# jaymarichua/Applestar

Hardware: AMD Instinct MI355X
Metric: learner samples/sec (AlphaStar policy) (higher is better)
Workload: dtype fp32

## Files before the change

applestar_amd/csrc/bindings.cpp:

```cpp
#include <cstring>
#include <cstdlib>
#include <map>
#include <string>
#include <torch/extension.h>
#include <c10/hip/HIPStream.h>
#include <c10/hip/HIPGuard.h>

#include "kernels.h"

namespace {

hipStream_t stream() { return c10::hip::getCurrentHIPStream().stream(); }

int dt(const at::Tensor& t) {
  if (t.scalar_type() == at::kFloat) return as::DT_F32;
  if (t.scalar_type() == at::kBFloat16) return as::DT_BF16;
  TORCH_CHECK(false, "applestar_amd: unsupported dtype ", t.scalar_type());
}

void check_cuda(const at::Tensor& t, const char* name) {
  TORCH_CHECK(t.is_cuda(), "applestar_amd: ", name, " must be a GPU tensor");
  TORCH_CHECK(t.is_contiguous(), "applestar_amd: ", name, " must be contiguous");
}

// ... 1634 lines not shown
  TORCH_CHECK(dy.dim() == 2, "wgrad: dy [R, N]");
  TORCH_CHECK(dy.is_contiguous() && x.is_contiguous(), "wgrad: dy and x must be contiguous");
  const int64_t R = dy.size(0), N = dy.size(1);
  int64_t K, H = 1, W = 1;
  if (cin > 0) {
    TORCH_CHECK(x.dim() == 4 && x.size(3) == cin && x.size(0) * x.size(1) * x.size(2) == R, "wgrad: x NHWC");
    H = x.size(1);
    W = x.size(2);
    K = 9 * cin;
    TORCH_CHECK(cin % 8 == 0, "wgrad: Cin % 8");
  } else {
    TORCH_CHECK(x.dim() == 2 && x.size(0) == R, "wgrad: x [R, K]");
    K = x.size(1);
  }
  TORCH_CHECK(N % 8 == 0 && K % 8 == 0, "wgrad: N and K must be multiples of 8");
  TORCH_CHECK(R * N * 2 < 0x7ffffff0LL && x.numel() * 2 < 0x7ffffff0LL, "wgrad: tensor too large");
  c10::hip::HIPGuard g(dy.device().index());
  const int S = R > 0 ? as::wgrad_splits(R, static_cast<int>(N), static_cast<int>(K)) : 1;
  auto opts = dy.options().dtype(at::kFloat);
  if (R == 0) {
    auto zo = bf16_out ? dy.options() : opts;
    return {at::zeros({N, K}, zo), want_bias ? at::zeros({N}, zo) : at::Tensor()};
  }
  const int64_t NK = N * K, stride = NK + (want_bias ? N : 0);
  if (bf16_out && S == 1) {
    auto flat = at::empty({stride}, dy.options());
    as::wgrad(dy.data_ptr(), x.data_ptr(), reinterpret_cast<float*>(flat.data_ptr()),
              want_bias ? reinterpret_cast<float*>(static_cast<at::BFloat16*>(flat.data_ptr()) + NK) : nullptr, 0, R,
              static_cast<int>(N), static_cast<int>(K), static_cast<int>(H), static_cast<int>(W), static_cast<int>(cin),
              1, stream(), true);
    return {flat.narrow(0, 0, NK).view({N, K}), want_bias ? flat.narrow(0, NK, N) : at::Tensor()};
  }
  auto part = at::empty({S, stride}, opts);
  static const bool nan_fill = [] {
    const char* e = std::getenv("APPLESTAR_WGRAD_NANFILL");
    return e != nullptr && e[0] == '1';
  }();
  if (nan_fill) part.fill_(std::numeric_limits<float>::quiet_NaN());
  as::wgrad(dy.data_ptr(), x.data_ptr(), part.data_ptr<float>(), want_bias ? part.data_ptr<float>() + NK : nullptr,
            stride, R, static_cast<int>(N), static_cast<int>(K), static_cast<int>(H), static_cast<int>(W),
            static_cast<int>(cin), S, stream());
  at::Tensor flat;
  if (bf16_out && S <= 1024) {
    flat = at::empty({stride}, dy.options());
    as::column_reduce_bf16(part.data_ptr<float>(), flat.data_ptr(), S, static_cast<int>(stride), stream());
  } else if (S == 1) {
    flat = part.view({stride});
  } else {
    flat = at::empty({stride}, opts);
    as::column_reduce(part.data_ptr<float>(), flat.data_ptr<float>(), S, static_cast<int>(stride), stream());
  }
  if (bf16_out && flat.scalar_type() != at::kBFloat16) flat = flat.to(at::kBFloat16);
  return {flat.narrow(0, 0, NK).view({N, K}), want_bias ? flat.narrow(0, NK, N) : at::Tensor()};
}

namespace {
int idx_code(const at::Tensor& t) {
  if (t.scalar_type() == at::kShort) return 0;
  if (t.scalar_type() == at::kInt) return 1;
  TORCH_CHECK(t.scalar_type() == at::kLong, "bo_encoder: index dtype int16 / int32 / int64");
  return 2;
}

as::BoWeights bo_weights(const std::vector<at::Tensor>& p, int* wdt) {
  TORCH_CHECK(p.size() == 2 + 12 * as::kBoLayers, "bo_encoder: 38 parameter tensors");
  const auto lin_t = p[0].scalar_type();
  TORCH_CHECK(lin_t == at::kFloat || lin_t == at::kBFloat16, "bo_encoder: linear dtype");
  auto lin = [&](const at::Tensor& t, int64_t numel) {
    TORCH_CHECK(t.is_cuda() && t.is_contiguous() && t.scalar_type() == lin_t && t.numel() == numel,
                "bo_encoder: linear parameter (dtype / shape / contiguity)");
    return static_cast<const void*>(t.data_ptr());
  };
  auto ln = [&](const at::Tensor& t) {
    TORCH_CHECK(t.is_cuda() && t.is_contiguous() && t.scalar_type() == at::kFloat && t.numel() == 64,
                "bo_encoder: LayerNorm parameter fp32 [64]");
    return t.data_ptr<float>();
  };
  as::BoWeights w;
  w.w0 = lin(p[0], 64 * 214);
  w.b0 = lin(p[1], 64);
  for (int l = 0; l < as::kBoLayers; ++l) {
    const int o = 2 + 12 * l;
    w.ln1w[l] = ln(p[o]);
    w.ln1b[l] = ln(p[o + 1]);
    w.wqkv[l] = lin(p[o + 2], 48 * 64);
    w.bqkv[l] = lin(p[o + 3], 48);
    w.wp[l] = lin(p[o + 4], 64 * 16);
    w.bp[l] = lin(p[o + 5], 64);
    w.ln2w[l] = ln(p[o + 6]);
    w.ln2b[l] = ln(p[o + 7]);
    w.w1[l] = lin(p[o + 8], 128 * 64);
    w.b1[l] = lin(p[o + 9], 128);
    w.w2[l] = lin(p[o + 10], 64 * 128);
    w.b2[l] = lin(p[o + 11], 64);
  }
  *wdt = lin_t == at::kBFloat16 ? as::DT_BF16 : as::DT_F32;
  return w;
}
}

std::vector<at::Tensor> bo_encoder_fwd(const at::Tensor& bo, const at::Tensor& loc, const std::vector<at::Tensor>& params,
                                       bool save) {
  check_cuda(bo, "bo");
  check_cuda(loc, "loc");
  TORCH_CHECK(bo.dim() == 2 && bo.size(1) == as::kBoTokens && bo.is_contiguous() && loc.sizes() == bo.sizes() &&
                  loc.is_contiguous() && loc.scalar_type() == bo.scalar_type(),
// ... 966 lines not shown
  m.def("varlen_attn_fwd_f32", &varlen_attn_fwd_f32);
  m.def("conv3x3_f32_epi2", &conv3x3_f32_epi2);
  m.def("conv3x3_f32_epi2_supported", &conv3x3_f32_epi2_supported);
  m.def("conv3x3_f32", &conv3x3_f32);
  m.def("fused_clip_adam", &fused_clip_adam);
  m.def("head_sample", &head_sample);
  m.def("target_unit_sample", &target_unit_sample);
  m.def("fused_adam_chunk", &as::fused_adam_chunk);
  m.def("wgrad_f32", &wgrad_f32, py::arg("dy"), py::arg("x"), py::arg("cin"), py::arg("want_bias"),
        py::arg("out") = py::none());
  m.def("gemm_f32", &gemm_f32);
  m.def("gemm_bf16_small", &gemm_bf16_small);
  m.def("gemm_bf16", &gemm_bf16);
  m.def("small_gemm", &small_gemm);
  m.def("small_wgrad", &small_wgrad);
  m.def("small_gemm_splitk", &small_gemm_splitk);
  m.def("f32_mfma_mode", &as::f32_mfma_mode);
  m.def("set_f32_pipe_variant", &as::set_f32_pipe_variant);
  m.def("set_f32_conv_variant", &as::set_f32_conv_variant);
  m.def("set_f32_mfma_mode", &as::set_f32_mfma_mode);
  m.def("conv3x3_f32_supported", &as::conv3x3_f32_supported);
  m.def("varlen_attn_bwd_f32", &varlen_attn_bwd_f32);
  m.def("attn_f32_variant", [](int64_t v) { return static_cast<int64_t>(as::attn_f32_variant(static_cast<int>(v))); });
  m.def("su_sample", &su_sample);
  m.def("segment_copy", &segment_copy);
  m.def("conv_wt", &conv_wt);
  m.def("upconv1_fwd", &upconv1_fwd);
  m.def("upconv1_bwd", &upconv1_bwd, py::arg("x_nhwc"), py::arg("w"), py::arg("dy"), py::arg("relu_mask") = false);
  m.def("maxpool2_fwd", &maxpool2_fwd);
  m.def("maxpool2_bwd", &maxpool2_bwd, py::arg("dy"), py::arg("pos"), py::arg("H"), py::arg("W"),
        py::arg("mask") = py::none());
  m.def("maxpool2_bwd_relu", &maxpool2_bwd_relu);
  m.def("spatial_embed_pool_fwd", &spatial_embed_pool_fwd, py::arg("planes"), py::arg("effects"), py::arg("w_dense"),
        py::arg("bias"), py::arg("rows"), py::arg("ex"), py::arg("ey"), py::arg("entity_num"),
        py::arg("ordered") = false);
  m.def("spatial_pool_supported", [](int64_t h, int64_t w) { return as::spatial_pool_supported(static_cast<int>(h), static_cast<int>(w)); });
  m.def("segment_sum", &segment_sum);
  m.def("spatial_dense_wgrad_pooled", &spatial_dense_wgrad_pooled);
  m.def("spatial_gather_rows_pooled", &spatial_gather_rows_pooled);
  m.def("entity_mean_pool", &entity_mean_pool);
  m.def("table_grad", &table_grad, py::arg("src"), py::arg("idx"), py::arg("V"), py::arg("ordered") = false);
  m.def("gather_steps_fwd", &gather_steps_fwd);
  m.def("gather_steps_bwd", &gather_steps_bwd);
  m.def("scatter_conn_fwd", &scatter_conn_fwd);
  m.def("scatter_conn_bwd", &scatter_conn_bwd);
  m.def("conv3x3_fwd", &conv3x3_fwd);
  m.def("wgrad", &wgrad, py::arg("dy"), py::arg("x"), py::arg("cin"), py::arg("want_bias"),
        py::arg("bf16_out") = false);
  m.def("pointwise_conv", &pointwise_conv);
  m.def("pointwise_supported", [](int64_t ci, int64_t co) { return as::pointwise_supported(static_cast<int>(ci), static_cast<int>(co)); });
  m.def("lstm_split_error", &lstm_split_error);
  m.def("lstm_split_flag", &lstm_split_flag);
  m.def("multi_copy", &multi_copy);
  m.def("ln_affine_grads", &ln_affine_grads);
  m.def("multi_strided_copy", &multi_strided_copy);
  m.def("multi_accumulate", &multi_accumulate);
  m.def("multi_strided_accumulate", &multi_strided_accumulate);
  m.def("loc_in_fwd", &loc_in_fwd);
  m.def("vsp_fwd", &vsp_fwd);
  m.def("rl_loss", &rl_loss, py::arg("alp"), py::arg("blp"), py::arg("hm"), py::arg("ent"), py::arg("kl"), py::arg("v"),
        py::arg("r"), py::arg("wm"), py::arg("atflag"), py::arg("sc"), py::arg("upgo_f"), py::arg("only_value"),
        py::arg("ordered") = false, py::arg("sk") = py::none(), py::arg("dflag") = py::none());
  m.def("sl_ce_fwd", &sl_ce_fwd, py::arg("logits"), py::arg("labels"), py::arg("eps"), py::arg("row_on") = py::none(),
        py::arg("su_len") = py::none(), py::arg("su_on") = py::none(), py::arg("S") = 1, py::arg("su_mask") = false);
  m.def("sl_ce_bwd", &sl_ce_bwd, py::arg("logits"), py::arg("labels"), py::arg("eps"), py::arg("row_on"),
        py::arg("su_len"), py::arg("su_on"), py::arg("S"), py::arg("su_mask"), py::arg("stats"), py::arg("grad"));
  m.def("sl_loss_tail", &sl_loss_tail, py::arg("losses"), py::arg("argmaxes"), py::arg("labels"), py::arg("masks"),
        py::arg("su_loss"), py::arg("su_labels"), py::arg("su_len"), py::arg("su_on"), py::arg("preds"),
        py::arg("ent_num"), py::arg("w"), py::arg("cr_scale"), py::arg("n"));
  m.def("sl_ce_su_max_c", []() { return as::sl_ce_su_max_c(); });
  m.def("gate_chain", &gate_chain);
  m.def("gate_chain_f32", &gate_chain_f32);
  m.def("vsp_pool_fwd", &vsp_pool_fwd);
  m.def("vsp_pool_bwd", &vsp_pool_bwd);
  m.def("vsp_in_channels", []() { return as::vsp_in_channels(); });
  m.def("vsp_out_channels", []() { return as::vsp_out_channels(); });
  m.def("vsp_bwd", &vsp_bwd);
  m.def("loc_in_supported", [](int64_t c, int64_t p) { return as::loc_in_supported(static_cast<int>(c), static_cast<int>(p)); });
  m.def("loc_in_bwd", &loc_in_bwd);
  m.def("head_stats_fwd", &head_stats_fwd, py::arg("logits"), py::arg("teacher"), py::arg("action"),
        py::arg("successive") = py::none());
  m.def("resmlp_fwd", &resmlp_fwd);
  m.def("resmlp_bwd", &resmlp_bwd);
  m.def("bo_encoder_fwd", &bo_encoder_fwd);
  m.def("bo_encoder_bwd", &bo_encoder_bwd, py::arg("bo"), py::arg("loc"), py::arg("params"), py::arg("save"),
        py::arg("dmean"), py::arg("ordered") = false);
  m.def("head_stats_bwd", &head_stats_bwd, py::arg("logits"), py::arg("teacher"), py::arg("action"), py::arg("stats"),
        py::arg("grad"), py::arg("successive") = py::none());
  m.def("act_grad_nhwc", &act_grad_nhwc);
  m.def("conv3x3_supported", [](int64_t cin, int64_t cout) { return as::conv3x3_supported(static_cast<int>(cin), static_cast<int>(cout)); });
}
```

applestar_amd/csrc/kernels.h:

```cpp
#pragma once
#include <hip/hip_runtime.h>
#include <stdint.h>

namespace as {

enum DType : int { DT_F32 = 0, DT_BF16 = 1 };
enum SrcType : int { SRC_U8 = 0, SRC_I8 = 1, SRC_I16 = 2, SRC_I32 = 3, SRC_I64 = 4, SRC_F16 = 5, SRC_F32 = 6 };
enum FieldKind : int { FIELD_ONE_HOT = 0, FIELD_BINARY = 1, FIELD_SCALAR = 2 };

constexpr int kMaxFields = 40;
struct EntityFields {
  const void* ptr[kMaxFields];
  int dtype[kMaxFields];
  int kind[kMaxFields];
  int offset[kMaxFields];
  int width[kMaxFields];
  int n;
};

void layer_norm_fwd(const void* x, int x_dt, const void* res, int res_dt, const float* w, const float* b,
                    void* y, int y_dt, float* xsum, float* mean, float* rstd, long rows, int cols, float eps,
                    int act, hipStream_t s);
void layer_norm_bwd(const void* dy, int dy_dt, const void* xin, int xin_dt, const void* y, int y_dt,
                    const float* w, const float* mean, const float* rstd, void* dx, int dx_dt,
                    float* dw_part, float* db_part, long rows, int cols, int act, int nblk, hipStream_t s,
                    const float* msrc = nullptr, float* dxm = nullptr);
void column_reduce(float* part, float* out, int nrows, int cols, hipStream_t s);
void entity_pack(const void* num, bool num64, int B, int N, long total, bool* valid, int64_t* flat, int64_t* seg,
                 int* cu, hipStream_t s);
void embed_relu_fwd(const void* table, int dt, const void* idx, int idt, void* out, long U, int V, int D,
                    hipStream_t s);
void embed_relu_bwd(const void* dout, const void* out, int dt, const void* idx, int idt, float* dtab, long U, int V,
                    int D, bool direct, hipStream_t s);
void column_reduce_bf16(const float* part, void* out, int nrows, int cols, hipStream_t s);
int layer_norm_bwd_blocks(long rows);

void reverse_scan(const float* a, const float* b, const float* init, float* y, int K, int T, int B,
                  hipStream_t s);

void gated_residual_fwd(const void* y, const void* g, const float* sp, const void* x, const void* post, void* out,
                        int dt, long n, hipStream_t s);
int vsp_in_channels();
int vsp_out_channels();
void vsp_fwd(const void* sc, const void* own, const void* enemy, const float* w, const float* b, void* out, long P,
             hipStream_t s, int dt = DT_BF16);
int vsp_bwd_blocks(long P);
void vsp_pool_fwd(const void* sc, const void* own, const void* enemy, const float* w, const float* b, void* pooled,
                  uint8_t* pos, int B, int H, int W, hipStream_t s, int dt = DT_BF16);
void vsp_pool_bwd(const void* dpooled, const uint8_t* pos, const void* pooled, const void* sc, const void* own,
                  const void* enemy, const float* w, void* dsc, float* part, int B, int H, int W, int nblk,
                  hipStream_t s, int dt = DT_BF16);
void vsp_bwd(const void* dout, const void* out, const void* sc, const void* own, const void* enemy, const float* w,
             void* dsc, float* part, long P, int nblk, hipStream_t s, int dt = DT_BF16);
bool loc_in_supported(int C, int P);
void loc_in_fwd(const void* y0, const void* p, const float* wp, void* out, long npix, int HW, hipStream_t s);
int loc_in_bwd_blocks(long npix);
void loc_in_bwd(const void* dy, const void* y, const void* p, const float* wp, void* dym, void* dp, float* part,
                long npix, int HW, int nblk, hipStream_t s);
void gated_residual_bwd(const void* dout, const void* y, const void* g, const float* sp, const void* out,
                        const void* xin, int dt, void* dy, void* dg, void* dx, float* dsp_part, long n, int nblk,
                        hipStream_t s);
int elementwise_blocks(long n);

bool lnlstm_supported(int H);
struct LstmSplit {
  unsigned long long* slab;
  int* err;
};
void lnlstm_fwd(const float* xp, const float* h0, const float* c0, const void* wT, int w_dt, const float* lnh_w,
                const float* lnh_b, const float* lnc_w, const float* lnc_b, int T, int B, int H, float eps, float* out,
                float* c_all, float* xhat_h, float* rstd_h, float* gates, float* xhat_c, float* rstd_c, float* hT,
                float* cT, hipStream_t s, const LstmSplit* split = nullptr, unsigned short* out_bf16 = nullptr);
void lnlstm_bwd(const float* dout, const float* dhT, const float* dcT, const float* gates, const float* c_all,
                const float* xhat_c, const float* rstd_c, const float* xhat_h, const float* rstd_h, const void* w,
                int w_dt, const float* lnh_w, const float* lnc_w, int T, int B, int H, float* dgates, float* dhg,
                float* dc_ln, float* dh0, float* dc0, hipStream_t s, const LstmSplit* split = nullptr);

void entity_embed_fwd(const EntityFields& f, const int64_t* index, const void* wT, int w_dt, const float* bias,
                      void* out, int out_dt, long T, hipStream_t s);
int entity_wgrad_chunks(long T);
void entity_embed_wgrad(const EntityFields& f, const int64_t* index, const void* dout, const void* out, int dt,
                        float* part, long T, int K_in, int nchunk, hipStream_t s);
void entity_onehot(const EntityFields& f, const int64_t* index, void* X, int x_dt, long T, int K_in, hipStream_t s);

struct SpatialPlanes {
  const uint8_t* height;
  const uint8_t* plane[6];
// ... 88 lines not shown
bool conv3x3_f32_supported(int Cin, int Cout);
void conv3x3_f32_fwd(const float* x, const float* w, const float* bias, const float* res, float* out, int B, int H,
                     int W, int Cin, int Cout, int act, hipStream_t s);
bool conv3x3_f32_epi2_supported(int Cin, int Cout);
void conv3x3_f32_fwd_epi2(const float* x, const float* w, const float* res, const float* res2, long res2_rows,
                          const float* mask, float* out, int B, int H, int W, int Cin, int Cout, hipStream_t s);
int wgrad_f32_splits(long R, int N, int K);
void set_f32_pipe_variant(int v);
int f32_conv_variant();
void set_f32_conv_variant(int v);
int f32_mfma_mode();
void set_f32_mfma_mode(int mode);
void small_nt(const void* a, const void* b, const float* bias, const void* res, const void* amask, int mask_mode,
              void* out, long M, int N, int K, int act, bool bf16, hipStream_t s);
int small_nt_splits(long M, int N, int K);
void small_nt_splitk(const void* a, const void* b, const float* bias, float* part, int S, void* out, long M, int N,
                     int K, int act, bool bf16, hipStream_t s);
void small_tn(const void* dy, const void* x, const void* ymask, int mask_mode, void* dw, void* db, long R, int N,
              int K, bool bf16_in, bool bf16_out, hipStream_t s);
void gemm_bf16_small(const void* a, const void* b, const float* bias, const void* res, void* out, long M, int N, int K,
                     int act, hipStream_t s);
bool gemm_f32_is_small(long M, int N);
void gemm_bf16(const void* a, const void* b, const float* bias, const void* res, void* out, long M, int N, int K,
               int act, hipStream_t s);
void gemm_f32(const float* a, const float* b, const float* bias, const float* res, float* out, long M, int N, int K,
              int act, hipStream_t s);
void wgrad_f32(const float* dy, const float* x, float* dw_part, float* db_part, long part_stride, long R, int N, int K,
               int H, int W, int Cin, int S, hipStream_t st);
int conv_wgrad_halo_f32_mode();
void set_conv_wgrad_halo_f32_mode(int mode);
bool conv_wgrad_f32_halo_supported(int N, int H, int W, int Cin);
bool conv_wgrad_f32_halo_selected(int N, int H, int W, int Cin);
int conv_wgrad_f32_splits(long R, int N, int K, int H, int W, int Cin);
void conv_wgrad_f32_halo(const float* dy, const float* x, float* dw_part, float* db_part, long part_stride, long R,
                         int N, int K, int H, int W, int Cin, int S, long rows_per_split, hipStream_t st);

void head_sample(const void* logits, int logits_dt, long ld_logits, int B, int C, float inv_t, const uint8_t* mask,
                 long mask_ld, const int64_t* lens, const float* u, const void* table, int table_dt,
                 const float* tbias, int D, float* out_logits, int64_t* action, float* emb, hipStream_t s);
void target_unit_sample(const void* e, int e_dt, const float* w1, const float* b1, const float* w2, const float* b2,
                        const void* key, int key_dt, int B, int N, const int64_t* lens, float inv_t, const float* u,
                        float* out_logits, int64_t* action, hipStream_t s);

int fused_adam_chunk();
void fused_clip_adam(const void* table, const long* chunks, int nchunks, int ntensors, float* part,
                     const float* gate, float* norm_out, float max_norm, float* mom, float* scale, float* mom_init,
                     const float* hp, float lr_bc1, float b1, float b2, float inv_sqrt_bc2, float eps, float wd,
                     int decoupled, hipStream_t s);

int wgrad_splits(long R, int N, int K);

constexpr int kCopyMaxT = 64;
constexpr long kCopyChunk = 8192;
constexpr long kCopyRawChunk = 16384;
struct CopyArgs {
  int ntensors;
  int chunk_start[kCopyMaxT + 1];
  const void* src[kCopyMaxT];
  void* dst[kCopyMaxT];
  long n[kCopyMaxT];
  unsigned char dts[kCopyMaxT];
};
void multi_copy(const CopyArgs& a, hipStream_t s);
void multi_accumulate(const CopyArgs& a, float scale, hipStream_t s);

constexpr int kColMaxP = 32;
struct ColSumArgs {
  int npieces;
  long rows;
  int block_start[kColMaxP + 1];
  float* dst[kColMaxP];
  int dld[kColMaxP], doff[kColMaxP], width[kColMaxP], nsrc[kColMaxP];
  const float* src[kColMaxP][3];
  int sld[kColMaxP][3], soff[kColMaxP][3];
};
void col_sum(const ColSumArgs& a, hipStream_t s);

constexpr int kLogpMaxH = 8;
struct LogpArgs {
  int nheads;
  long row_start[kLogpMaxH + 1];
  const void* logits[kLogpMaxH];
  const int64_t* action[kLogpMaxH];
  float* out[kLogpMaxH];
  int cols[kLogpMaxH];
  unsigned char bf16[kLogpMaxH];
  long blk_start[kLogpMaxH + 1];
  unsigned char big[kLogpMaxH];
};
void multi_logp(const LogpArgs& a, hipStream_t s);

long presplit_b_bytes(int N, int K);
void presplit_b(const float* b, int N, int K, bool trans, void* out, hipStream_t s);
bool gemm_f32_psb_supported(long M, int N, int K);
constexpr int kPresplitMax = 48;
struct PresplitArgs {
  int n;
  int block_start[kPresplitMax + 1];
  const float* src[kPresplitMax];
  void* dst[kPresplitMax];
  int N[kPresplitMax], K[kPresplitMax];
  unsigned char trans[kPresplitMax];
};
void multi_presplit(const PresplitArgs& a, hipStream_t s);
void gemm_f32_psb(const float* a, const void* bsplit, const float* bias, const float* res, float* out, long M, int N,
                  int K, int act, int variant, hipStream_t s);
bool gemm_f32_psb_planes_supported(long M, int N, int K);
// ... 173 lines not shown
```

applestar_amd/csrc/kernels/multi_copy.hip:

```cpp
#include "../common.h"
#include "../kernels.h"

namespace as {
namespace {

__device__ __forceinline__ float copy_src(const void* src, long i, unsigned char dts) {
  if (dts & 8) return static_cast<float>(static_cast<const unsigned char*>(src)[i]);
  if (dts & 16) return static_cast<float>(static_cast<const short*>(src)[i]);
  return (dts & 1) ? static_cast<const float*>(src)[i] : bf2f(static_cast<const bf16_t*>(src)[i]);
}

__global__ __launch_bounds__(256) void multi_copy_kernel(const CopyArgs a) {
  const int b = blockIdx.x;
  int t = 0;
  while (t + 1 < a.ntensors && a.chunk_start[t + 1] <= b) ++t;
  const void* src = a.src[t];
  void* dst = a.dst[t];
  if (a.dts[t] & 4) {
    const long i0 = static_cast<long>(b - a.chunk_start[t]) * kCopyRawChunk;
    const long i1 = i0 + kCopyRawChunk < a.n[t] ? i0 + kCopyRawChunk : a.n[t];
    const auto* s8 = static_cast<const unsigned char*>(src);
    auto* d8 = static_cast<unsigned char*>(dst);
    if (((reinterpret_cast<uintptr_t>(src) | reinterpret_cast<uintptr_t>(dst) | a.n[t]) & 15) == 0) {
      constexpr int U = static_cast<int>(kCopyRawChunk / (16 * 256));
      if (i1 - i0 == kCopyRawChunk) {
        uint4 v[U];
#pragma unroll
        for (int u = 0; u < U; ++u) v[u] = *reinterpret_cast<const uint4*>(s8 + i0 + 16 * (threadIdx.x + 256 * u));
#pragma unroll
        for (int u = 0; u < U; ++u) *reinterpret_cast<uint4*>(d8 + i0 + 16 * (threadIdx.x + 256 * u)) = v[u];
        return;
      }
      for (long i = i0 + 16 * threadIdx.x; i < i1; i += 16 * 256)
        *reinterpret_cast<uint4*>(d8 + i) = *reinterpret_cast<const uint4*>(s8 + i);
    } else {
      for (long i = i0 + threadIdx.x; i < i1; i += 256) d8[i] = s8[i];
    }
    return;
  }
  const long i0 = static_cast<long>(b - a.chunk_start[t]) * kCopyChunk;
  const long i1 = i0 + kCopyChunk < a.n[t] ? i0 + kCopyChunk : a.n[t];
  const bool df = (a.dts[t] & 2) != 0;
  const unsigned char dts = a.dts[t];
  if (i1 - i0 == kCopyChunk) {
    constexpr int U = static_cast<int>(kCopyChunk / 256);
    float v[U];
#pragma unroll
    for (int u = 0; u < U; ++u) v[u] = copy_src(src, i0 + threadIdx.x + 256 * u, dts);
#pragma unroll
    for (int u = 0; u < U; ++u) {
      const long i = i0 + threadIdx.x + 256 * u;
      if (df) static_cast<float*>(dst)[i] = v[u];
      else static_cast<bf16_t*>(dst)[i] = f2bf(v[u]);
    }
    return;
  }
  for (long i = i0 + threadIdx.x; i < i1; i += 256) {
    const float v = copy_src(src, i, dts);
    if (df) static_cast<float*>(dst)[i] = v;
    else static_cast<bf16_t*>(dst)[i] = f2bf(v);
  }
}

__device__ __forceinline__ float acc_op(float d, float s, float scale) {
#pragma clang fp contract(off)
  const float t = d + s;
  return t * scale;
}

__device__ __forceinline__ float acc_src(const float* p, long i) { return p[i]; }
__device__ __forceinline__ float acc_src(const bf16_t* p, long i) { return bf2f(p[i]); }

__device__ __forceinline__ void acc_unpack(const uint4& w, float (&v)[4], const float*) {
  v[0] = __uint_as_float(w.x), v[1] = __uint_as_float(w.y), v[2] = __uint_as_float(w.z), v[3] = __uint_as_float(w.w);
}
__device__ __forceinline__ void acc_unpack(const uint4& w, float (&v)[8], const bf16_t*) {
  const uint32_t u[4] = {w.x, w.y, w.z, w.w};
#pragma unroll
  for (int k = 0; k < 4; ++k) {
    v[2 * k] = __uint_as_float(u[k] << 16);
    v[2 * k + 1] = __uint_as_float(u[k] & 0xffff0000u);
  }
}

template <typename S>
__device__ __forceinline__ void acc_chunk(float* dst, const S* src, long i0, long i1, float scale) {
  constexpr int V = 16 / static_cast<int>(sizeof(S));
  constexpr int Q = V / 4;
  if (((reinterpret_cast<uintptr_t>(src) | reinterpret_cast<uintptr_t>(dst)) & 15) == 0) {
    if (i1 - i0 == kCopyChunk) {
      constexpr int U = static_cast<int>(kCopyChunk / (256 * V));
      uint4 sw[U];
      f32x4 dv[U][Q];
#pragma unroll
      for (int u = 0; u < U; ++u) {
        const long i = i0 + static_cast<long>(V) * (threadIdx.x + 256 * u);
        sw[u] = *reinterpret_cast<const uint4*>(src + i);
#pragma unroll
        for (int q = 0; q < Q; ++q) dv[u][q] = *reinterpret_cast<const f32x4*>(dst + i + 4 * q);
      }
#pragma unroll
      for (int u = 0; u < U; ++u) {
        const long i = i0 + static_cast<long>(V) * (threadIdx.x + 256 * u);
        float sv[V];
        acc_unpack(sw[u], sv, src);
#pragma unroll
        for (int q = 0; q < Q; ++q) {
          f32x4 r;
#pragma unroll
          for (int k = 0; k < 4; ++k) r[k] = acc_op(dv[u][q][k], sv[4 * q + k], scale);
          *reinterpret_cast<f32x4*>(dst + i + 4 * q) = r;
        }
      }
      return;
    }
    const long nw = (i1 - i0) / V;
    for (long w = threadIdx.x; w < nw; w += 256) {
      const long i = i0 + w * V;
      const uint4 s4 = *reinterpret_cast<const uint4*>(src + i);
      f32x4 d4[Q];
#pragma unroll
      for (int q = 0; q < Q; ++q) d4[q] = *reinterpret_cast<const f32x4*>(dst + i + 4 * q);
      float sv[V];
      acc_unpack(s4, sv, src);
#pragma unroll
      for (int q = 0; q < Q; ++q) {
        f32x4 r;
#pragma unroll
        for (int k = 0; k < 4; ++k) r[k] = acc_op(d4[q][k], sv[4 * q + k], scale);
        *reinterpret_cast<f32x4*>(dst + i + 4 * q) = r;
      }
    }
    for (long i = i0 + nw * V + threadIdx.x; i < i1; i += 256) dst[i] = acc_op(dst[i], acc_src(src, i), scale);
    return;
// ... 168 lines not shown
```

applestar_amd/csrc/kernels/pool_reduce.hip:

```cpp
#include <algorithm>

#include "../common.h"
#include "../kernels.h"

namespace as {
namespace {

struct V8 {
  float v[8];
};

template <typename T> __device__ __forceinline__ V8 load8(const T* p);
template <> __device__ __forceinline__ V8 load8<bf16_t>(const bf16_t* p) {
  const uint4 u = *reinterpret_cast<const uint4*>(p);
  const uint32_t w[4] = {u.x, u.y, u.z, u.w};
  V8 r;
#pragma unroll
  for (int j = 0; j < 4; ++j) {
    r.v[2 * j] = __uint_as_float(w[j] << 16);
    r.v[2 * j + 1] = __uint_as_float(w[j] & 0xffff0000u);
  }
  return r;
}
template <> __device__ __forceinline__ V8 load8<float>(const float* p) {
  const float4 a = *reinterpret_cast<const float4*>(p);
  const float4 b = *reinterpret_cast<const float4*>(p + 4);
  V8 r;
  r.v[0] = a.x; r.v[1] = a.y; r.v[2] = a.z; r.v[3] = a.w;
  r.v[4] = b.x; r.v[5] = b.y; r.v[6] = b.z; r.v[7] = b.w;
  return r;
}

template <typename T> __device__ __forceinline__ void store8(T* p, const V8& r);
template <> __device__ __forceinline__ void store8<bf16_t>(bf16_t* p, const V8& r) {
  uint4 u;
  u.x = f2bf2(r.v[0], r.v[1]);
  u.y = f2bf2(r.v[2], r.v[3]);
  u.z = f2bf2(r.v[4], r.v[5]);
  u.w = f2bf2(r.v[6], r.v[7]);
  *reinterpret_cast<uint4*>(p) = u;
}
template <> __device__ __forceinline__ void store8<float>(float* p, const V8& r) {
  *reinterpret_cast<float4*>(p) = make_float4(r.v[0], r.v[1], r.v[2], r.v[3]);
  *reinterpret_cast<float4*>(p + 4) = make_float4(r.v[4], r.v[5], r.v[6], r.v[7]);
}

int grid_for(long n) {
  long b = (n + 255) / 256;
  return static_cast<int>(b < 1 ? 1 : (b > 16384 ? 16384 : b));
}

template <typename T>
__global__ __launch_bounds__(256) void maxpool2_fwd_kernel(const T* __restrict__ x, T* __restrict__ y,
// ... 164 lines not shown
    const long v = static_cast<long>(num[i]);
    return v < 0 ? 0L : (v > N ? static_cast<long>(N) : v);
  };
  if (threadIdx.x < 64) {
    long acc = 0;
    for (int i = threadIdx.x; i < b; i += 64) acc += len_of(i);
    acc = wave_sum_long(acc);
    if (threadIdx.x == 0) {
      base_s = acc;
      cu[b] = static_cast<int>(acc);
      if (b == B - 1) cu[B] = static_cast<int>(acc + len_of(b));
    }
  }
  __syncthreads();
  const long base = base_s, len = len_of(b);
  for (int j = threadIdx.x; j < N; j += 256) {
    valid[static_cast<long>(b) * N + j] = j < len;
    const long k = base + j;
    if (j < len && k < total) {
      flat[k] = static_cast<int64_t>(b) * N + j;
      seg[k] = b;
    }
  }
}

template <typename OutT>
__global__ __launch_bounds__(1024) void column_reduce_kernel(const float* __restrict__ part, OutT* __restrict__ out,
                                                             int nrows, int cols, long rstride) {
  __shared__ float red[16][64];
  const int c = blockIdx.x * 64 + (threadIdx.x & 63);
  const int g = threadIdx.x >> 6;
  float s0 = 0.f, s1 = 0.f, s2 = 0.f, s3 = 0.f;
  if (c < cols) {
    int r = g;
    for (; r + 48 < nrows; r += 64) {
      s0 += part[static_cast<long>(r) * rstride + c];
      s1 += part[static_cast<long>(r + 16) * rstride + c];
      s2 += part[static_cast<long>(r + 32) * rstride + c];
      s3 += part[static_cast<long>(r + 48) * rstride + c];
    }
    for (; r < nrows; r += 16) s0 += part[static_cast<long>(r) * rstride + c];
  }
  red[g][threadIdx.x & 63] = (s0 + s1) + (s2 + s3);
  __syncthreads();
  if (g == 0 && c < cols) {
    float s = 0.f;
#pragma unroll
    for (int k = 0; k < 16; ++k) s += red[k][threadIdx.x];
    if constexpr (sizeof(OutT) == 2) out[c] = f2bf(s);
    else out[c] = s;
  }
}

__global__ __launch_bounds__(256) void column_reduce_chunk_kernel(float* __restrict__ part, int nrows, int cols) {
  __shared__ float red[4][64];
  const int c = blockIdx.x * 64 + (threadIdx.x & 63);
  const int g = threadIdx.x >> 6;
  const int r0 = blockIdx.y * 256, r1 = min(r0 + 256, nrows);
  float s0 = 0.f, s1 = 0.f, s2 = 0.f, s3 = 0.f;
  if (c < cols) {
    int r = r0 + g;
    for (; r + 12 < r1; r += 16) {
      s0 += part[static_cast<long>(r) * cols + c];
      s1 += part[static_cast<long>(r + 4) * cols + c];
      s2 += part[static_cast<long>(r + 8) * cols + c];
      s3 += part[static_cast<long>(r + 12) * cols + c];
    }
    for (; r < r1; r += 4) s0 += part[static_cast<long>(r) * cols + c];
  }
  red[g][threadIdx.x & 63] = (s0 + s1) + (s2 + s3);
  __syncthreads();
  if (g == 0 && c < cols)
    part[static_cast<long>(r0) * cols + c] = (red[0][threadIdx.x] + red[1][threadIdx.x]) +
                                             (red[2][threadIdx.x] + red[3][threadIdx.x]);
}


constexpr int kAffRows = 512;
__global__ __launch_bounds__(256) void ln_affine_grads_kernel(const float* __restrict__ dy, const float* __restrict__ xh,
                                                              float* __restrict__ part, long R, int C) {
  __shared__ float sw[4][64], sb[4][64];
  const int lane = threadIdx.x & 63, w = threadIdx.x >> 6;
  const int c = blockIdx.x * 64 + lane;
  const long r0 = static_cast<long>(blockIdx.y) * kAffRows;
  const long r1 = r0 + kAffRows < R ? r0 + kAffRows : R;
  float aw = 0.f, ab = 0.f;
  if (c < C) {
#pragma unroll 4
    for (long r = r0 + w; r < r1; r += 4) {
      const float g = dy[r * C + c];
      aw += g * xh[r * C + c];
      ab += g;
    }
  }
  sw[w][lane] = aw;
  sb[w][lane] = ab;
  __syncthreads();
  if (w == 0 && c < C) {
    float* o = part + static_cast<long>(blockIdx.y) * 2 * C;
    o[c] = (sw[0][lane] + sw[1][lane]) + (sw[2][lane] + sw[3][lane]);
    o[C + c] = (sb[0][lane] + sb[1][lane]) + (sb[2][lane] + sb[3][lane]);
  }
}
}

namespace {
__global__ __launch_bounds__(256) void maxpool2_bwd_relu_kernel(const bf16_t* __restrict__ dy,
                                                                const uint8_t* __restrict__ pos,
                                                                const bf16_t* __restrict__ y, bf16_t* __restrict__ dx,
                                                                int B, int H, int W, int C) {
  const int Ho = H >> 1, Wo = W >> 1, C8 = C >> 3;
  const int total = B * Ho * Wo * C8;
  for (int i = blockIdx.x * blockDim.x + threadIdx.x; i < total; i += gridDim.x * blockDim.x) {
    const int c8 = i % C8;
    int r = i / C8;
    const int ox = r % Wo;
    r /= Wo;
    const int oy = r % Ho;
    const int b = r / Ho;
    const long oi = static_cast<long>(i) * 8;
    const uint4 g = *reinterpret_cast<const uint4*>(dy + oi);
    const uint4 yv = *reinterpret_cast<const uint4*>(y + oi);
    const uint2 pp = *reinterpret_cast<const uint2*>(pos + oi);
    const uint32_t gw[4] = {g.x, g.y, g.z, g.w}, yw[4] = {yv.x, yv.y, yv.z, yv.w};
    uint32_t outw[4][4];
#pragma unroll
    for (int t = 0; t < 4; ++t)
#pragma unroll
      for (int j = 0; j < 4; ++j) outw[t][j] = 0u;
// ... 163 lines not shown
    case 0: { using I = int64_t; BODY; } break;                    \
    case 1: { using I = int32_t; BODY; } break;                    \
    case 2: { using I = int16_t; BODY; } break;                    \
    case 3: { using I = uint8_t; BODY; } break;                    \
    default: { using I = int8_t; BODY; } break;                    \
  }

void embed_relu_fwd(const void* table, int dt, const void* idx, int idt, void* out, long U, int V, int D,
                    hipStream_t s) {
  const long n = U * D;
  if (n == 0) return;
  const unsigned blocks = static_cast<unsigned>(std::min<long>((n + 255) / 256, 1024));
  if (dt == DT_BF16) {
    AS_EMB_IDX(idt, hipLaunchKernelGGL((embed_relu_fwd_kernel<bf16_t, I>), dim3(blocks), dim3(256), 0, s,
                                       static_cast<const bf16_t*>(table), static_cast<const I*>(idx),
                                       static_cast<bf16_t*>(out), U, V, D))
  } else {
    AS_EMB_IDX(idt, hipLaunchKernelGGL((embed_relu_fwd_kernel<float, I>), dim3(blocks), dim3(256), 0, s,
                                       static_cast<const float*>(table), static_cast<const I*>(idx),
                                       static_cast<float*>(out), U, V, D))
  }
}

void embed_relu_bwd(const void* dout, const void* out, int dt, const void* idx, int idt, float* dtab, long U, int V,
                    int D, bool direct, hipStream_t s) {
  const long n = U * D;
  long blocks = direct ? 1 : std::min<long>(std::max<long>((n + 1023) / 1024, 1), 256);
  const size_t lds = static_cast<size_t>(V) * D * sizeof(float);
  if (dt == DT_BF16) {
    AS_EMB_IDX(idt, hipLaunchKernelGGL((embed_relu_bwd_kernel<bf16_t, I>), dim3(static_cast<unsigned>(blocks)),
                                       dim3(256), lds, s, static_cast<const bf16_t*>(dout),
                                       static_cast<const bf16_t*>(out), static_cast<const I*>(idx), dtab, U, V, D,
                                       direct ? 1 : 0))
  } else {
    AS_EMB_IDX(idt, hipLaunchKernelGGL((embed_relu_bwd_kernel<float, I>), dim3(static_cast<unsigned>(blocks)),
                                       dim3(256), lds, s, static_cast<const float*>(dout),
                                       static_cast<const float*>(out), static_cast<const I*>(idx), dtab, U, V, D,
                                       direct ? 1 : 0))
  }
}
#undef AS_EMB_IDX

void entity_pack(const void* num, bool num64, int B, int N, long total, bool* valid, int64_t* flat, int64_t* seg,
                 int* cu, hipStream_t s) {
  if (B == 0) return;
  if (num64)
    hipLaunchKernelGGL(entity_pack_kernel<int64_t>, dim3(B), dim3(256), 0, s, static_cast<const int64_t*>(num), B, N,
                       total, valid, flat, seg, cu);
  else
    hipLaunchKernelGGL(entity_pack_kernel<int>, dim3(B), dim3(256), 0, s, static_cast<const int*>(num), B, N, total,
                       valid, flat, seg, cu);
}

void column_reduce(float* part, float* out, int nrows, int cols, hipStream_t s) {
  if (nrows <= 1024) {
    hipLaunchKernelGGL(column_reduce_kernel<float>, dim3((cols + 63) / 64), dim3(1024), 0, s, part, out, nrows, cols,
                       static_cast<long>(cols));
    return;
  }
  const int nchunk = (nrows + 255) / 256;
  hipLaunchKernelGGL(column_reduce_chunk_kernel, dim3((cols + 63) / 64, nchunk), dim3(256), 0, s, part, nrows,
                     cols);
  hipLaunchKernelGGL(column_reduce_kernel<float>, dim3((cols + 63) / 64), dim3(1024), 0, s, part, out, nchunk, cols,
                     256L * cols);
}

void column_reduce_bf16(const float* part, void* out, int nrows, int cols, hipStream_t s) {
  hipLaunchKernelGGL(column_reduce_kernel<bf16_t>, dim3((cols + 63) / 64), dim3(1024), 0, s, part,
                     static_cast<bf16_t*>(out), nrows, cols, static_cast<long>(cols));
}

int ln_affine_slices(long R) { return static_cast<int>((R + kAffRows - 1) / kAffRows); }

void ln_affine_grads(const float* dy, const float* xh, float* part, long R, int C, hipStream_t s) {
  const int S = ln_affine_slices(R);
  if (S == 0 || C == 0) return;
  hipLaunchKernelGGL(ln_affine_grads_kernel, dim3((C + 63) / 64, S), dim3(256), 0, s, dy, xh, part, R, C);
}

}
```

Measured before the change: 8527.

## Vectorize multi_copy chunks and add opt-in vectorized column reduce kernels

Rewrites the raw byte-copy path of multi_copy to choose the widest aligned word type (16/8/4/2/1 bytes) with unrolled passes, and doubles the raw chunk size. Adds a vectorized typed-copy path for full aligned chunks that loads 16-byte words and unpacks them. Adds float4-vectorized column reduction kernels with strided rows, but they only run when an environment variable or setter enables them, and exposes column_reduce to Python. The larger raw chunk means fewer blocks for mid-sized tensors.

```diff
diff --git a/applestar_amd/csrc/bindings.cpp b/applestar_amd/csrc/bindings.cpp
--- a/applestar_amd/csrc/bindings.cpp
+++ b/applestar_amd/csrc/bindings.cpp
@@ -1710,6 +1710,33 @@
   }
   if (bf16_out && flat.scalar_type() != at::kBFloat16) flat = flat.to(at::kBFloat16);
   return {flat.narrow(0, 0, NK).view({N, K}), want_bias ? flat.narrow(0, NK, N) : at::Tensor()};
+}
+
+at::Tensor column_reduce(const at::Tensor& part, const c10::optional<at::Tensor>& out, bool bf16_out) {
+  TORCH_CHECK(part.is_cuda() && part.scalar_type() == at::kFloat && part.dim() == 2, "column_reduce: part fp32 [rows, cols]");
+  const int64_t rows = part.size(0), cols = part.size(1);
+  TORCH_CHECK(rows >= 1 && cols >= 1 && rows < (1 << 30) && cols < (1 << 30), "column_reduce: empty or too large");
+  TORCH_CHECK(part.stride(1) == 1 && (rows == 1 || part.stride(0) >= cols), "column_reduce: rows must be dense");
+  TORCH_CHECK(!bf16_out || rows <= 1024, "column_reduce: bf16 output takes at most 1024 rows");
+  c10::hip::HIPGuard g(part.device().index());
+  const auto odt = bf16_out ? at::kBFloat16 : at::kFloat;
+  at::Tensor o;
+  if (out && out->defined()) {
+    TORCH_CHECK(out->scalar_type() == odt && out->is_contiguous() && out->numel() == cols &&
+                out->device() == part.device(), "column_reduce: out must be a contiguous [cols] buffer of the output dtype");
+    o = *out;
+  } else {
+    o = at::empty({cols}, part.options().dtype(odt));
+  }
+  const at::Tensor src = rows > 1024 ? part.clone(at::MemoryFormat::Contiguous) : part;
+  const int64_t rstride = rows == 1 ? cols : src.stride(0);
+  if (bf16_out)
+    as::column_reduce_bf16(src.data_ptr<float>(), o.data_ptr(), static_cast<int>(rows), static_cast<int>(cols), stream(),
+                           rstride);
+  else
+    as::column_reduce(src.data_ptr<float>(), o.data_ptr<float>(), static_cast<int>(rows), static_cast<int>(cols),
+                      stream(), rstride);
+  return o;
 }
 
 namespace {
@@ -2782,6 +2809,9 @@
   m.def("lstm_split_error", &lstm_split_error);
   m.def("lstm_split_flag", &lstm_split_flag);
   m.def("multi_copy", &multi_copy);
+  m.def("column_reduce", &column_reduce, py::arg("part"), py::arg("out") = py::none(), py::arg("bf16_out") = false);
+  m.def("column_reduce_mode", &as::column_reduce_mode);
+  m.def("set_column_reduce_mode", &as::set_column_reduce_mode);
   m.def("ln_affine_grads", &ln_affine_grads);
   m.def("multi_strided_copy", &multi_strided_copy);
   m.def("multi_accumulate", &multi_accumulate);
diff --git a/applestar_amd/csrc/kernels.h b/applestar_amd/csrc/kernels.h
--- a/applestar_amd/csrc/kernels.h
+++ b/applestar_amd/csrc/kernels.h
@@ -25,14 +25,16 @@
                     const float* w, const float* mean, const float* rstd, void* dx, int dx_dt,
                     float* dw_part, float* db_part, long rows, int cols, int act, int nblk, hipStream_t s,
                     const float* msrc = nullptr, float* dxm = nullptr);
-void column_reduce(float* part, float* out, int nrows, int cols, hipStream_t s);
+void column_reduce(float* part, float* out, int nrows, int cols, hipStream_t s, long rstride = 0);
 void entity_pack(const void* num, bool num64, int B, int N, long total, bool* valid, int64_t* flat, int64_t* seg,
                  int* cu, hipStream_t s);
 void embed_relu_fwd(const void* table, int dt, const void* idx, int idt, void* out, long U, int V, int D,
                     hipStream_t s);
 void embed_relu_bwd(const void* dout, const void* out, int dt, const void* idx, int idt, float* dtab, long U, int V,
                     int D, bool direct, hipStream_t s);
-void column_reduce_bf16(const float* part, void* out, int nrows, int cols, hipStream_t s);
+void column_reduce_bf16(const float* part, void* out, int nrows, int cols, hipStream_t s, long rstride = 0);
+int column_reduce_mode();
+void set_column_reduce_mode(int mode);
 int layer_norm_bwd_blocks(long rows);
 
 void reverse_scan(const float* a, const float* b, const float* init, float* y, int K, int T, int B,
@@ -227,7 +229,7 @@
 
 constexpr int kCopyMaxT = 64;
 constexpr long kCopyChunk = 8192;
-constexpr long kCopyRawChunk = 16384;
+constexpr long kCopyRawChunk = 32768;
 struct CopyArgs {
   int ntensors;
   int chunk_start[kCopyMaxT + 1];
diff --git a/applestar_amd/csrc/kernels/multi_copy.hip b/applestar_amd/csrc/kernels/multi_copy.hip
--- a/applestar_amd/csrc/kernels/multi_copy.hip
+++ b/applestar_amd/csrc/kernels/multi_copy.hip
@@ -8,6 +8,92 @@
   if (dts & 8) return static_cast<float>(static_cast<const unsigned char*>(src)[i]);
   if (dts & 16) return static_cast<float>(static_cast<const short*>(src)[i]);
   return (dts & 1) ? static_cast<const float*>(src)[i] : bf2f(static_cast<const bf16_t*>(src)[i]);
+}
+
+__device__ __forceinline__ float acc_op(float d, float s, float scale) {
+#pragma clang fp contract(off)
+  const float t = d + s;
+  return t * scale;
+}
+
+__device__ __forceinline__ float acc_src(const float* p, long i) { return p[i]; }
+__device__ __forceinline__ float acc_src(const bf16_t* p, long i) { return bf2f(p[i]); }
+
+__device__ __forceinline__ void acc_unpack(const uint4& w, float (&v)[4], const float*) {
+  v[0] = __uint_as_float(w.x), v[1] = __uint_as_float(w.y), v[2] = __uint_as_float(w.z), v[3] = __uint_as_float(w.w);
+}
+__device__ __forceinline__ void acc_unpack(const uint4& w, float (&v)[8], const bf16_t*) {
+  const uint32_t u[4] = {w.x, w.y, w.z, w.w};
+#pragma unroll
+  for (int k = 0; k < 4; ++k) {
+    v[2 * k] = __uint_as_float(u[k] << 16);
+    v[2 * k + 1] = __uint_as_float(u[k] & 0xffff0000u);
+  }
+}
+
+__device__ __forceinline__ void acc_unpack(const uint4& w, float (&v)[16], const unsigned char*) {
+  const uint32_t u[4] = {w.x, w.y, w.z, w.w};
+#pragma unroll
+  for (int k = 0; k < 16; ++k) v[k] = static_cast<float>((u[k >> 2] >> (8 * (k & 3))) & 0xffu);
+}
+__device__ __forceinline__ void acc_unpack(const uint4& w, float (&v)[8], const short*) {
+  const uint32_t u[4] = {w.x, w.y, w.z, w.w};
+#pragma unroll
+  for (int k = 0; k < 8; ++k) v[k] = static_cast<float>(static_cast<short>((u[k >> 1] >> (16 * (k & 1))) & 0xffffu));
+}
+
+typedef uint32_t u32x4 __attribute__((ext_vector_type(4)));
+typedef uint32_t u32x2 __attribute__((ext_vector_type(2)));
+
+template <typename W, int U>
+__device__ __forceinline__ void raw_pass(W* d, const W* s) {
+  W v[U];
+#pragma unroll
+  for (int u = 0; u < U; ++u) v[u] = s[threadIdx.x + 256 * u];
+#pragma unroll
+  for (int u = 0; u < U; ++u) d[threadIdx.x + 256 * u] = v[u];
+}
+
+template <typename W>
+__device__ __forceinline__ void raw_chunk(unsigned char* d8, const unsigned char* s8, long nbytes) {
+  const W* s = reinterpret_cast<const W*>(s8);
+  W* d = reinterpret_cast<W*>(d8);
+  const int n = static_cast<int>(nbytes / static_cast<long>(sizeof(W)));
+  int i = 0;
+  for (; i + 256 * 8 <= n; i += 256 * 8) raw_pass<W, 8>(d + i, s + i);
+  if (i + 256 * 4 <= n) { raw_pass<W, 4>(d + i, s + i); i += 256 * 4; }
+  if (i + 256 * 2 <= n) { raw_pass<W, 2>(d + i, s + i); i += 256 * 2; }
+  if (i + 256 <= n) { raw_pass<W, 1>(d + i, s + i); i += 256; }
+  if (i + static_cast<int>(threadIdx.x) < n) d[i + threadIdx.x] = s[i + threadIdx.x];
+}
+
+template <typename S>
+__device__ __forceinline__ void copy_chunk_vec(void* dst, const S* src, long i0, bool df) {
+  constexpr int V = 16 / static_cast<int>(sizeof(S));
+  constexpr int U = static_cast<int>(kCopyChunk / (256 * V));
+  uint4 w[U];
+#pragma unroll
+  for (int u = 0; u < U; ++u) w[u] = *reinterpret_cast<const uint4*>(src + i0 + V * (threadIdx.x + 256 * u));
+#pragma unroll
+  for (int u = 0; u < U; ++u) {
+    const long i = i0 + V * (threadIdx.x + 256 * u);
+    float v[V];
+    acc_unpack(w[u], v, src);
+    if (df) {
+#pragma unroll
+      for (int q = 0; q < V / 4; ++q)
+        *reinterpret_cast<f32x4*>(static_cast<float*>(dst) + i + 4 * q) =
+            f32x4{v[4 * q], v[4 * q + 1], v[4 * q + 2], v[4 * q + 3]};
+    } else if constexpr (V == 4) {
+      *reinterpret_cast<uint2*>(static_cast<bf16_t*>(dst) + i) = make_uint2(f2bf2(v[0], v[1]), f2bf2(v[2], v[3]));
+    } else {
+#pragma unroll
+      for (int q = 0; q < V / 8; ++q)
+        *reinterpret_cast<uint4*>(static_cast<bf16_t*>(dst) + i + 8 * q) =
+            make_uint4(f2bf2(v[8 * q], v[8 * q + 1]), f2bf2(v[8 * q + 2], v[8 * q + 3]),
+                       f2bf2(v[8 * q + 4], v[8 * q + 5]), f2bf2(v[8 * q + 6], v[8 * q + 7]));
+    }
+  }
 }
 
 __global__ __launch_bounds__(256) void multi_copy_kernel(const CopyArgs a) {
@@ -21,21 +107,12 @@
     const long i1 = i0 + kCopyRawChunk < a.n[t] ? i0 + kCopyRawChunk : a.n[t];
     const auto* s8 = static_cast<const unsigned char*>(src);
     auto* d8 = static_cast<unsigned char*>(dst);
-    if (((reinterpret_cast<uintptr_t>(src) | reinterpret_cast<uintptr_t>(dst) | a.n[t]) & 15) == 0) {
-      constexpr int U = static_cast<int>(kCopyRawChunk / (16 * 256));
-      if (i1 - i0 == kCopyRawChunk) {
-        uint4 v[U];
-#pragma unroll
-        for (int u = 0; u < U; ++u) v[u] = *reinterpret_cast<const uint4*>(s8 + i0 + 16 * (threadIdx.x + 256 * u));
-#pragma unroll
-        for (int u = 0; u < U; ++u) *reinterpret_cast<uint4*>(d8 + i0 + 16 * (threadIdx.x + 256 * u)) = v[u];
-        return;
-      }
-      for (long i = i0 + 16 * threadIdx.x; i < i1; i += 16 * 256)
-        *reinterpret_cast<uint4*>(d8 + i) = *reinterpret_cast<const uint4*>(s8 + i);
-    } else {
-      for (long i = i0 + threadIdx.x; i < i1; i += 256) d8[i] = s8[i];
-    }
+    const uintptr_t m = reinterpret_cast<uintptr_t>(src) | reinterpret_cast<uintptr_t>(dst) | static_cast<uintptr_t>(a.n[t]);
+    if ((m & 15) == 0) raw_chunk<u32x4>(d8 + i0, s8 + i0, i1 - i0);
+    else if ((m & 7) == 0) raw_chunk<u32x2>(d8 + i0, s8 + i0, i1 - i0);
+    else if ((m & 3) == 0) raw_chunk<uint32_t>(d8 + i0, s8 + i0, i1 - i0);
+    else if ((m & 1) == 0) raw_chunk<unsigned short>(d8 + i0, s8 + i0, i1 - i0);
+    else raw_chunk<unsigned char>(d8 + i0, s8 + i0, i1 - i0);
     return;
   }
   const long i0 = static_cast<long>(b - a.chunk_start[t]) * kCopyChunk;
@@ -43,6 +120,13 @@
   const bool df = (a.dts[t] & 2) != 0;
   const unsigned char dts = a.dts[t];
   if (i1 - i0 == kCopyChunk) {
+    if (((reinterpret_cast<uintptr_t>(src) | reinterpret_cast<uintptr_t>(dst)) & 15) == 0) {
+      if (dts & 8) copy_chunk_vec(dst, static_cast<const unsigned char*>(src), i0, df);
+      else if (dts & 16) copy_chunk_vec(dst, static_cast<const short*>(src), i0, df);
+      else if (dts & 1) copy_chunk_vec(dst, static_cast<const float*>(src), i0, df);
+      else copy_chunk_vec(dst, static_cast<const bf16_t*>(src), i0, df);
+      return;
+    }
     constexpr int U = static_cast<int>(kCopyChunk / 256);
     float v[U];
 #pragma unroll
@@ -59,27 +143,6 @@
     const float v = copy_src(src, i, dts);
     if (df) static_cast<float*>(dst)[i] = v;
     else static_cast<bf16_t*>(dst)[i] = f2bf(v);
-  }
-}
-
-__device__ __forceinline__ float acc_op(float d, float s, float scale) {
-#pragma clang fp contract(off)
-  const float t = d + s;
-  return t * scale;
-}
-
-__device__ __forceinline__ float acc_src(const float* p, long i) { return p[i]; }
-__device__ __forceinline__ float acc_src(const bf16_t* p, long i) { return bf2f(p[i]); }
-
-__device__ __forceinline__ void acc_unpack(const uint4& w, float (&v)[4], const float*) {
-  v[0] = __uint_as_float(w.x), v[1] = __uint_as_float(w.y), v[2] = __uint_as_float(w.z), v[3] = __uint_as_float(w.w);
-}
-__device__ __forceinline__ void acc_unpack(const uint4& w, float (&v)[8], const bf16_t*) {
-  const uint32_t u[4] = {w.x, w.y, w.z, w.w};
-#pragma unroll
-  for (int k = 0; k < 4; ++k) {
-    v[2 * k] = __uint_as_float(u[k] << 16);
-    v[2 * k + 1] = __uint_as_float(u[k] & 0xffff0000u);
   }
 }
 
diff --git a/applestar_amd/csrc/kernels/pool_reduce.hip b/applestar_amd/csrc/kernels/pool_reduce.hip
--- a/applestar_amd/csrc/kernels/pool_reduce.hip
+++ b/applestar_amd/csrc/kernels/pool_reduce.hip
@@ -1,4 +1,6 @@
 #include <algorithm>
+#include <cstdlib>
+#include <type_traits>
 
 #include "../common.h"
 #include "../kernels.h"
@@ -269,7 +271,8 @@
   }
 }
 
-__global__ __launch_bounds__(256) void column_reduce_chunk_kernel(float* __restrict__ part, int nrows, int cols) {
+__global__ __launch_bounds__(256) void column_reduce_chunk_kernel(float* __restrict__ part, int nrows, int cols,
+                                                                  long rstride) {
   __shared__ float red[4][64];
   const int c = blockIdx.x * 64 + (threadIdx.x & 63);
   const int g = threadIdx.x >> 6;
@@ -278,20 +281,118 @@
   if (c < cols) {
     int r = r0 + g;
     for (; r + 12 < r1; r += 16) {
-      s0 += part[static_cast<long>(r) * cols + c];
-      s1 += part[static_cast<long>(r + 4) * cols + c];
-      s2 += part[static_cast<long>(r + 8) * cols + c];
-      s3 += part[static_cast<long>(r + 12) * cols + c];
-    }
-    for (; r < r1; r += 4) s0 += part[static_cast<long>(r) * cols + c];
+      s0 += part[static_cast<long>(r) * rstride + c];
+      s1 += part[static_cast<long>(r + 4) * rstride + c];
+      s2 += part[static_cast<long>(r + 8) * rstride + c];
+      s3 += part[static_cast<long>(r + 12) * rstride + c];
+    }
+    for (; r < r1; r += 4) s0 += part[static_cast<long>(r) * rstride + c];
   }
   red[g][threadIdx.x & 63] = (s0 + s1) + (s2 + s3);
   __syncthreads();
   if (g == 0 && c < cols)
-    part[static_cast<long>(r0) * cols + c] = (red[0][threadIdx.x] + red[1][threadIdx.x]) +
+    part[static_cast<long>(r0) * rstride + c] = (red[0][threadIdx.x] + red[1][threadIdx.x]) +
                                              (red[2][threadIdx.x] + red[3][threadIdx.x]);
 }
 
+constexpr int kColLoads = 8;
+
+__device__ __forceinline__ f32x4 ld4(const float* p) { return *reinterpret_cast<const f32x4*>(p); }
+
+template <int N, typename Idx, typename Add>
+__device__ __forceinline__ void col4_rows(const float* __restrict__ p, long gs, Idx&& idx, Add&& add) {
+  f32x4 v[N];
+#pragma unroll
+  for (int u = 0; u < N; ++u) v[u] = ld4(p + idx(u) * gs);
+#pragma unroll
+  for (int u = 0; u < N; ++u) add(u, v[u]);
+}
+
+template <typename F>
+__device__ __forceinline__ void col4_rest(int n, F&& f) {
+  switch (n) {
+#define AS_COL_CASE(N) case N: f(std::integral_constant<int, N>{}); break;
+    AS_COL_CASE(1) AS_COL_CASE(2) AS_COL_CASE(3) AS_COL_CASE(4) AS_COL_CASE(5)
+    AS_COL_CASE(6) AS_COL_CASE(7) AS_COL_CASE(8) AS_COL_CASE(9) AS_COL_CASE(10)
+#undef AS_COL_CASE
+    default: break;
+  }
+}
+
+template <int J>
+__device__ __forceinline__ f32x4 col4_group_sum(const float* __restrict__ p, int n, long gs, int j) {
+  const int K = n >> 2, T = n & 3;
+  const f32x4 zero = {0.f, 0.f, 0.f, 0.f};
+  if constexpr (J == 4) {
+    f32x4 s = zero;
+    int t = 0;
+    for (; t + kColLoads <= K; t += kColLoads)
+      col4_rows<kColLoads>(p, gs, [&](int u) { return 4 * (t + u) + j; }, [&](int, const f32x4& v) { s += v; });
+    const int reg = K - t;
+    col4_rest(reg + (j == 0 ? T : 0), [&](auto nc) {
+      col4_rows<decltype(nc)::value>(
+          p, gs, [&](int u) { return u < reg ? 4 * (t + u) + j : 4 * K + (u - reg); },
+          [&](int, const f32x4& v) { s += v; });
+    });
+    return s;
+  } else {
+    f32x4 s[4] = {zero, zero, zero, zero};
+    constexpr int SL = kColLoads / 4;
+    int k = 0;
+    for (; k + SL <= K; k += SL)
+      col4_rows<kColLoads>(p, gs, [&](int u) { return 4 * k + u; }, [&](int u, const f32x4& v) { s[u & 3] += v; });
+    col4_rest(n - 4 * k, [&](auto nc) {
+      constexpr int N = decltype(nc)::value;
+      col4_rows<N>(p, gs, [&](int u) { return 4 * k + u; },
+                   [&](int u, const f32x4& v) { s[u < (N & ~3) ? (u & 3) : 0] += v; });
+    });
+    return (s[0] + s[1]) + (s[2] + s[3]);
+  }
+}
+
+template <int G, int J>
+__device__ __forceinline__ void col4_partial(const float* __restrict__ part, long rstride, int r0, int r1, int cols,
+                                             float (*red)[64]) {
+  const int q = threadIdx.x & 15, g = (threadIdx.x >> 4) % G, j = threadIdx.x / (16 * G);
+  const int c = blockIdx.x * 64 + 4 * q;
+  const int left = r1 - r0 - g;
+  const int n = (c < cols && left > 0) ? (left + G - 1) / G : 0;
+  const f32x4 s = col4_group_sum<J>(part + static_cast<long>(r0 + g) * rstride + c, n, G * rstride, j);
+  *reinterpret_cast<f32x4*>(&red[g * J + j][4 * q]) = s;
+}
+
+template <typename OutT>
+__global__ __launch_bounds__(256) void column_reduce_vec_kernel(const float* __restrict__ part, OutT* __restrict__ out,
+                                                                int nrows, int cols, long rstride) {
+  __shared__ __attribute__((aligned(16))) float red[16][64];
+  col4_partial<16, 1>(part, rstride, 0, nrows, cols, red);
+  __syncthreads();
+  const int c = blockIdx.x * 64 + threadIdx.x;
+  if (threadIdx.x < 64 && c < cols) {
+    float s = 0.f;
+#pragma unroll
+    for (int k = 0; k < 16; ++k) s += red[k][threadIdx.x];
+    if constexpr (sizeof(OutT) == 2) out[c] = f2bf(s);
+    else out[c] = s;
+  }
+}
+
+__global__ __launch_bounds__(256) void column_reduce_chunk_vec_kernel(float* __restrict__ part, int nrows, int cols,
+                                                                      long rstride) {
+  __shared__ __attribute__((aligned(16))) float red[16][64];
+  const int r0 = blockIdx.y * 256, r1 = min(r0 + 256, nrows);
+  col4_partial<4, 4>(part, rstride, r0, r1, cols, red);
+  __syncthreads();
+  const int c = blockIdx.x * 64 + threadIdx.x;
+  if (threadIdx.x < 64 && c < cols) {
+    float grp[4];
+#pragma unroll
+    for (int k = 0; k < 4; ++k)
+      grp[k] = (red[4 * k][threadIdx.x] + red[4 * k + 1][threadIdx.x]) +
+               (red[4 * k + 2][threadIdx.x] + red[4 * k + 3][threadIdx.x]);
+    part[static_cast<long>(r0) * rstride + c] = (grp[0] + grp[1]) + (grp[2] + grp[3]);
+  }
+}
 
 constexpr int kAffRows = 512;
 __global__ __launch_bounds__(256) void ln_affine_grads_kernel(const float* __restrict__ dy, const float* __restrict__ xh,
@@ -561,22 +662,52 @@
                        valid, flat, seg, cu);
 }
 
-void column_reduce(float* part, float* out, int nrows, int cols, hipStream_t s) {
+int& column_reduce_ref() {
+  static int v = [] {
+    const char* e = std::getenv("APPLESTAR_COLUMN_REDUCE");
+    return (e != nullptr && e[0] == '1') ? 1 : 0;
+  }();
+  return v;
+}
+int column_reduce_mode() { return column_reduce_ref(); }
+void set_column_reduce_mode(int mode) { column_reduce_ref() = mode != 0 ? 1 : 0; }
+
+namespace {
+bool column_vec_ok(const float* part, int cols, long rstride) {
+  return column_reduce_ref() != 0 && cols % 4 == 0 && rstride % 4 == 0 && (reinterpret_cast<uintptr_t>(part) & 15) == 0;
+}
+
+bool column_vec_pays(int nrows, int cols) { return nrows <= 128 || (cols + 63) / 64 >= 1024; }
+
+template <typename OutT>
+void column_reduce_launch(const float* part, OutT* out, int nrows, int cols, long rstride, hipStream_t s) {
+  const dim3 grid((cols + 63) / 64);
+  if (column_vec_ok(part, cols, rstride) && column_vec_pays(nrows, cols))
+    hipLaunchKernelGGL(column_reduce_vec_kernel<OutT>, grid, dim3(256), 0, s, part, out, nrows, cols, rstride);
+  else
+    hipLaunchKernelGGL(column_reduce_kernel<OutT>, grid, dim3(1024), 0, s, part, out, nrows, cols, rstride);
+}
+}
+
+void column_reduce(float* part, float* out, int nrows, int cols, hipStream_t s, long rstride) {
+  if (cols <= 0) return;
+  if (rstride == 0) rstride = cols;
   if (nrows <= 1024) {
-    hipLaunchKernelGGL(column_reduce_kernel<float>, dim3((cols + 63) / 64), dim3(1024), 0, s, part, out, nrows, cols,
-                       static_cast<long>(cols));
+    column_reduce_launch(part, out, nrows, cols, rstride, s);
     return;
   }
   const int nchunk = (nrows + 255) / 256;
-  hipLaunchKernelGGL(column_reduce_chunk_kernel, dim3((cols + 63) / 64, nchunk), dim3(256), 0, s, part, nrows,
-                     cols);
-  hipLaunchKernelGGL(column_reduce_kernel<float>, dim3((cols + 63) / 64), dim3(1024), 0, s, part, out, nchunk, cols,
-                     256L * cols);
-}
-
-void column_reduce_bf16(const float* part, void* out, int nrows, int cols, hipStream_t s) {
-  hipLaunchKernelGGL(column_reduce_kernel<bf16_t>, dim3((cols + 63) / 64), dim3(1024), 0, s, part,
-                     static_cast<bf16_t*>(out), nrows, cols, static_cast<long>(cols));
+  const dim3 grid((cols + 63) / 64, nchunk);
+  if (column_vec_ok(part, cols, rstride))
+    hipLaunchKernelGGL(column_reduce_chunk_vec_kernel, grid, dim3(256), 0, s, part, nrows, cols, rstride);
+  else
+    hipLaunchKernelGGL(column_reduce_chunk_kernel, grid, dim3(256), 0, s, part, nrows, cols, rstride);
+  column_reduce_launch(part, out, nchunk, cols, 256L * rstride, s);
+}
+
+void column_reduce_bf16(const float* part, void* out, int nrows, int cols, hipStream_t s, long rstride) {
+  if (cols <= 0) return;
+  column_reduce_launch(part, static_cast<bf16_t*>(out), nrows, cols, rstride == 0 ? cols : rstride, s);
 }
 
 int ln_affine_slices(long R) { return static_cast<int>((R + kAffRows - 1) / kAffRows); }
```

Measured after the change: 8543, median of 6. No clear change (+0.2%).
